# francescofugazzi/3dgsconverter

Hardware: NVIDIA H100
Metric: Msplats/s SOR k=16 (higher is better)
Workload: dtype f32

## Files before the change

3dgsconverter_b200/csrc/gsx_sor.cu:

```cuda
#include "gsx_common.cuh"
#include "gsx_sor.cuh"

#include "gsx_radix.cuh"
#include <math.h>

namespace gsx {

#define GSX_D2LIM_BITS 0x60ad78ebu
#define GSX_FULL 0xffffffffu

#ifndef GSX_MORTON_BITS
#define GSX_MORTON_BITS 15
#endif
constexpr int kMortonBits = GSX_MORTON_BITS;
constexpr float kMortonScale = (float)(1 << (GSX_MORTON_BITS / 3));
constexpr float kMortonMax = kMortonScale - 1.f;
#ifndef GSX_SMALL_BUCKET
#define GSX_SMALL_BUCKET 64
#endif
constexpr int kSmallBucket = GSX_SMALL_BUCKET;
#ifndef GSX_QUERY_BATCH
#define GSX_QUERY_BATCH 16
#endif
constexpr int kQueryBatch = GSX_QUERY_BATCH;
// ... 1004 lines not shown
                                : "memory");
                        }
                        bar_phase ^= 1u;
                        if (__all_sync(GSX_FULL, ok != 0)) {
                            staged_s = s13;
                            staged_c = c13;
                        }
                    }
                }
#endif
            }
            if (STATS) {
                int tot = pc;
#pragma unroll
                for (int o = 16; o > 0; o >>= 1) tot += __shfl_xor_sync(GSX_FULL, tot, o);
                st_visits += (unsigned long long)tot;
                st_queries += 1;
            }
            TopK<NREG> tk;
            tk.init(K);

            unsigned pkey = 0xffffffffu;
            if (pc > 0) {
                float dx = fmaxf(fmaxf(__fsub_rn(blx, q.x), __fsub_rn(q.x, bhx)), 0.f);
                float dy = fmaxf(fmaxf(__fsub_rn(bly, q.y), __fsub_rn(q.y, bhy)), 0.f);
                float dz = fmaxf(fmaxf(__fsub_rn(blz, q.z), __fsub_rn(q.z, bhz)), 0.f);
                pkey = __float_as_uint(__fadd_rn(__fadd_rn(__fmul_rn(dx, dx), __fmul_rn(dy, dy)), __fmul_rn(dz, dz)));
            }

            int skip_chunk = -1;
            {
                int s13 = __shfl_sync(GSX_FULL, ps, 13), c13 = __shfl_sync(GSX_FULL, pc, 13);
                if (c13 > kSmallBucket && i >= s13 && i < (pos_t)s13 + c13) {
                    skip_chunk = (int)(i >> 5);
                    const pos_t j = ((pos_t)skip_chunk << 5) + lane;
                    scan32<NREG, STATS>(spos, j, j >= s13 && j < (pos_t)s13 + c13, q.x, q.y, q.z, tk, lane,
                                        st_scanned);
                }
            }

#pragma unroll 1
            for (;;) {
                const unsigned mp = __reduce_min_sync(GSX_FULL, pkey);
                if (mp == 0xffffffffu || !(__uint_as_float(mp) < tk.tau)) break;
                const int p = __ffs(__ballot_sync(GSX_FULL, pkey == mp)) - 1;
                if (lane == p) pkey = 0xffffffffu;
                const int s = __shfl_sync(GSX_FULL, ps, p), c = __shfl_sync(GSX_FULL, pc, p);
                const pos_t e = (pos_t)s + c;
                if (c <= kSmallBucket) {
#if GSX_KNN_TMA
                    const bool from_smem = staged_c > 0 && s == staged_s;
#pragma unroll 1
                    for (pos_t base = s; base < e; base += 32)
                        scan32<NREG, STATS>(spos, base + lane, base + lane < e, q.x, q.y, q.z, tk, lane, st_scanned,
                                            from_smem ? wbuf + (base - s) : nullptr);
#else
#pragma unroll 1
                    for (pos_t base = s; base < e; base += 32)
                        scan32<NREG, STATS>(spos, base + lane, base + lane < e, q.x, q.y, q.z, tk, lane, st_scanned);
#endif
                    continue;
                }
                const int skip = p == 13 ? skip_chunk : -1;
                const int fc = s >> 5, lc = (int)((e - 1) >> 5);
                const int fs = fc >> 5, ls = lc >> 5;
                auto chunk_group = [&](const int cbase) {
                    const int cid = cbase + lane;
                    const bool cv = cid >= fc && cid <= lc && cid != skip;
                    unsigned ckey = 0xffffffffu;
                    if (cv) {
                        float lb = box_lb(caabb, cid, q.x, q.y, q.z);
                        if (lb < tk.tau) ckey = __float_as_uint(lb);
                    }
                    if (STATS) st_boxes += __popc(__ballot_sync(GSX_FULL, cv));
                    for (;;) {
                        unsigned mc = __reduce_min_sync(GSX_FULL, ckey);
                        if (mc == 0xffffffffu || !(__uint_as_float(mc) < tk.tau)) break;
                        int srcc = __ffs(__ballot_sync(GSX_FULL, ckey == mc)) - 1;
                        if (lane == srcc) ckey = 0xffffffffu;
                        const pos_t j = ((pos_t)(cbase + srcc) << 5) + lane;
                        scan32<NREG, STATS>(spos, j, j >= s && j < e, q.x, q.y, q.z, tk, lane, st_scanned);
                    }
                };
#if GSX_KNN_FLAT_SUPERS > 0
                if (ls - fs < GSX_KNN_FLAT_SUPERS) {
                    for (int cb = fc; cb <= lc; cb += 32) chunk_group(cb);
                    continue;
                }
#endif
                for (int sb = fs; sb <= ls; sb += 32) {
                    const int sid = sb + lane;
                    unsigned skey = 0xffffffffu;
                    if (sid <= ls) {
                        float lb = box_lb(saabb, sid, q.x, q.y, q.z);
                        if (lb < tk.tau) skey = __float_as_uint(lb);
                    }
                    if (STATS) st_boxes += __popc(__ballot_sync(GSX_FULL, sid <= ls));
                    for (;;) {
                        unsigned ms = __reduce_min_sync(GSX_FULL, skey);
                        if (ms == 0xffffffffu || !(__uint_as_float(ms) < tk.tau)) break;
                        int srcs = __ffs(__ballot_sync(GSX_FULL, skey == ms)) - 1;
                        if (lane == srcs) skey = 0xffffffffu;
                        chunk_group((sb + srcs) * 32);
                    }
                }
            }

            const float d0 = __fsqrt_rn(tk.v0), d1 = NREG == 2 ? __fsqrt_rn(tk.v1) : 0.f;
            if (ES > 0) {
                float* row = epi + (int)(i - qb_p) * ES;
                if (ES <= 32) {
                    if (lane < ES) row[lane] = lane == ES - 1 ? q.w : d0;
                } else {
                    row[lane] = d0;
                    if (lane == 0) row[ES - 1] = q.w;
                }
                continue;
            }
            int valid = __popc(__ballot_sync(GSX_FULL, lane < K && d0 < 0.9e10f));
            if (NREG == 2) valid += __popc(__ballot_sync(GSX_FULL, lane + 32 < K && d1 < 0.9e10f));
            float sum = 0.f;
            for (int r = 0; r < valid; ++r) {
                float x = (NREG == 2 && r >= 32) ? __shfl_sync(GSX_FULL, d1, r - 32) : __shfl_sync(GSX_FULL, d0, r);
                sum = __fadd_rn(sum, x);
            }
            if (lane == 0) final_means[__float_as_int(q.w)] = valid > 0 ? __fdiv_rn(sum, (float)valid) : 0.f;
        }
        if (ES > 0) {
            __syncwarp();
            if (lane < (int)(qe - qb)) {
                const float* row = epi + lane * ES;
                float sum = 0.f;
                int valid = 0;
                for (int r = 0; r < K; ++r) {
                    const float x = row[r];
                    if (x < 0.9e10f) {
                        sum = __fadd_rn(sum, x);
                        ++valid;
                    }
                }
                final_means[__float_as_int(row[ES - 1])] = valid > 0 ? __fdiv_rn(sum, (float)valid) : 0.f;
            }
            __syncwarp();
        }
    }
    if (STATS && lane == 0) {
        atomicAdd(stats + 0, st_visits);
        atomicAdd(stats + 1, st_scanned);
        atomicAdd(stats + 2, st_boxes);
        atomicAdd(stats + 3, st_queries);
    }
}

#ifndef GSX_KNN16
#define GSX_KNN16 0
#endif
#include "gsx_sor_knn16.cuh"

__global__ void k_fill_f32(float* p, int64_t n, float v) {
    int64_t i = (int64_t)blockIdx.x * blockDim.x + threadIdx.x;
    if (i < n) p[i] = v;
}

template <int NREG, bool STATS, int ES>
static int launch_knn(SorWs& w, int64_t q_begin, int64_t q_end, int q_stride, int q_phase, int K, int hash_mode,
                      const float* bmin, float cell,
                      float* final_means, unsigned long long* stats, uint64_t M, int64_t want, cudaStream_t st) {
    int per_sm = 0;
    const size_t smem = (size_t)8 * kQueryBatch * ES * sizeof(float);
    GSX_CUDA_CHECK(cudaOccupancyMaxActiveBlocksPerMultiprocessor(&per_sm, k_sor_knn<NREG, STATS, ES>, 256, smem));
    int64_t grid = (int64_t)sm_count() * (per_sm > 0 ? per_sm : 4);
    if (grid > want) grid = want;
    if (grid < 1) grid = 1;
    k_sor_knn<NREG, STATS, ES><<<(int)grid, 256, smem, st>>>(w.spos, w.tab_se, w.tab_box, w.cellbits, w.caabb, w.saabb, final_means, w.counters,
                                                      q_begin, q_end, q_stride, q_phase, K, hash_mode, bmin[0], bmin[1],
                                                      bmin[2], cell,
                                                      (uint32_t)w.n, M, stats);
    return GSX_OK;
}

template <bool STATS>
static int launch_knn16(SorWs& w, int64_t q_begin, int64_t q_end, int q_stride, int q_phase, int K, int hash_mode,
                        const float* bmin, float cell, float* final_means, unsigned long long* stats, uint64_t M,
                        int64_t want, cudaStream_t st) {
    int per_sm = 0;
    GSX_CUDA_CHECK(cudaOccupancyMaxActiveBlocksPerMultiprocessor(&per_sm, k_sor_knn16<STATS>, 256, 0));
    int64_t grid = (int64_t)sm_count() * (per_sm > 0 ? per_sm : 4);
    want = (want + 1) / 2;
    if (grid > want) grid = want;
    if (grid < 1) grid = 1;
    k_sor_knn16<STATS><<<(int)grid, 256, 0, st>>>(w.spos, w.tab_se, w.tab_box, w.cellbits, w.caabb, w.saabb, final_means,
                                                  w.counters, q_begin, q_end, q_stride, q_phase, K, hash_mode, bmin[0],
                                                  bmin[1], bmin[2], cell, (uint32_t)w.n, M, stats);
    return GSX_OK;
}

#define GSX_STR2(x) #x
#define GSX_STR(x) GSX_STR2(x)
#if GSX_KNN_FLAT_SUPERS > 0
#define GSX_FLAT_INFO ";flat_supers=" GSX_STR(GSX_KNN_FLAT_SUPERS)
#else
#define GSX_FLAT_INFO ""
#endif
const char* sor_build_info() {
    return "knn=r02c"
           ";epi_smem=" GSX_STR(GSX_KNN_EPI_SMEM) ";first_sort=" GSX_STR(GSX_KNN_FIRST_SORT)
           ";query_batch=" GSX_STR(GSX_QUERY_BATCH) ";minblocks=" GSX_STR(GSX_KNN_MINBLOCKS)
           ";merge_threshold=" GSX_STR(GSX_MERGE_THRESHOLD) ";small_bucket=" GSX_STR(GSX_SMALL_BUCKET)
           GSX_FLAT_INFO ";knn16=" GSX_STR(GSX_KNN16) ";tma=" GSX_STR(GSX_KNN_TMA) ";i32=" GSX_STR(GSX_KNN_I32);
}

int sor_mean_dists(SorWs& w, int64_t q_begin, int64_t q_end, int q_stride, int q_phase, int k, int hash_mode,
                   const float* bmin, float cell,
                   float* final_means, unsigned long long* stats, cudaStream_t st) {
    GSX_NVTX("gsx::sor_mean_dists(k_sor_knn)");
    int64_t n = w.n;
    GSX_REQUIRE(k >= 1, GSX_ERR_ARG, "sor: k must be >= 1 (got %d)", k);
    GSX_REQUIRE(hash_mode == 0 || hash_mode == 1, GSX_ERR_ARG, "sor: bad hash_mode %d", hash_mode);
    GSX_REQUIRE(q_begin >= 0 && q_end <= n && q_begin <= q_end, GSX_ERR_ARG, "sor: bad query range");
    GSX_REQUIRE(q_stride >= 1 && q_phase >= 0 && q_phase < q_stride, GSX_ERR_ARG, "sor: bad query stride/phase");
    int K = k < 50 ? k : 50;
    if (q_end == q_begin) return GSX_OK;
    if (!(cell > 1e-8f)) {
        GSX_REQUIRE(q_begin == 0 && q_end == n, GSX_ERR_UNSUPPORTED, "sor: degenerate cell with a query range");
        k_fill_f32<<<(int)((n + 255) / 256), 256, 0, st>>>(final_means, n, 0.f);
        GSX_KERNEL_CHECK();
        return GSX_OK;
    }
    GSX_CUDA_CHECK(cudaMemsetAsync(w.counters, 0, sizeof(unsigned int), st));
    uint64_t M = 0xFFFFFFFFFFFFFFFFull / (uint64_t)n + 1ull;
    int64_t nq = (q_end - q_begin + q_stride - 1) / q_stride + kQueryBatch;
    int64_t want = (nq + (int64_t)kQueryBatch * 8 - 1) / ((int64_t)kQueryBatch * 8);
    int rc;
    if (GSX_KNN16 && K <= 16)
        rc = stats ? launch_knn16<true>(w, q_begin, q_end, q_stride, q_phase, K, hash_mode, bmin, cell, final_means, stats, M, want, st)
                   : launch_knn16<false>(w, q_begin, q_end, q_stride, q_phase, K, hash_mode, bmin, cell, final_means, stats, M, want, st);
    else {
#define GSX_KNN_ARGS w, q_begin, q_end, q_stride, q_phase, K, hash_mode, bmin, cell, final_means, stats, M, want, st
        constexpr int ES16 = GSX_KNN_EPI_SMEM ? 17 : 0, ES32 = GSX_KNN_EPI_SMEM ? 33 : 0;
        if (K <= 16) rc = stats ? launch_knn<1, true, ES16>(GSX_KNN_ARGS) : launch_knn<1, false, ES16>(GSX_KNN_ARGS);
        else if (K <= 32) rc = stats ? launch_knn<1, true, ES32>(GSX_KNN_ARGS) : launch_knn<1, false, ES32>(GSX_KNN_ARGS);
        else rc = stats ? launch_knn<2, true, 0>(GSX_KNN_ARGS) : launch_knn<2, false, 0>(GSX_KNN_ARGS);
#undef GSX_KNN_ARGS
    }
    if (rc) return rc;
    GSX_KERNEL_CHECK();
    return GSX_OK;
}

}
```

3dgsconverter_b200/csrc/gsx_sor_knn16.cuh:

```cuda

#ifndef GSX_MERGE16_THRESHOLD
#define GSX_MERGE16_THRESHOLD 4
#endif
#ifndef GSX_KNN16_MINBLOCKS
#define GSX_KNN16_MINBLOCKS 6
#endif

struct Lanes16 {
    int base;
    int hl;
    __device__ __forceinline__ unsigned ballot(bool p) const { return (__ballot_sync(GSX_FULL, p) >> base) & 0xffffu; }
    template <class T>
    __device__ __forceinline__ T bcast(T x, int src_hl) const { return __shfl_sync(GSX_FULL, x, src_hl, 16); }
    __device__ __forceinline__ unsigned hmin(unsigned x, bool& either) const {
        const unsigned lo = __reduce_min_sync(GSX_FULL, base ? 0xffffffffu : x);
        const unsigned hi = __reduce_min_sync(GSX_FULL, base ? x : 0xffffffffu);
        either = (lo & hi) != 0xffffffffu;
        return base ? hi : lo;
    }
};

struct TopK16 {
    float v;
    float tau;
    int K;
    __device__ __forceinline__ void init(int k) {
        K = k;
        v = tau = __uint_as_float(GSX_D2LIM_BITS);
    }
    __device__ __forceinline__ void refresh_tau(const Lanes16& L) { tau = L.bcast(v, K - 1); }
    __device__ __forceinline__ void insert(float x, const Lanes16& L) {
        float up = __shfl_up_sync(GSX_FULL, v, 1, 16);
        if (L.hl == 0) up = 0.f;
        if (v > x) v = fmaxf(up, x);
    }
    __device__ __forceinline__ void merge16(float nv, const Lanes16& L) {
        const int hl = L.hl;
#pragma unroll
        for (int k = 2; k <= 16; k <<= 1) {
#pragma unroll
            for (int j = k >> 1; j > 0; j >>= 1) {
                const float o = __shfl_xor_sync(GSX_FULL, nv, j);
                nv = (((hl & k) == 0) == ((hl & j) == 0)) ? fminf(nv, o) : fmaxf(nv, o);
            }
        }
        const float r = L.bcast(nv, 15 - hl);
        float m = fminf(v, r);
#pragma unroll
        for (int j = 8; j > 0; j >>= 1) {
            const float o = __shfl_xor_sync(GSX_FULL, m, j);
            m = ((hl & j) == 0) ? fminf(m, o) : fmaxf(m, o);
        }
        v = m;
    }
};

template <bool STATS>
__device__ __forceinline__ void scan16(const float4* __restrict__ spos, pos_t j, bool valid, float qx, float qy, float qz,
                                       TopK16& tk, const Lanes16& L, unsigned long long& n_scanned) {
    const float sentinel = __uint_as_float(GSX_D2LIM_BITS);
    float d2 = sentinel;
    if (valid) {
        const float4 c = __ldg(spos + j);
        const float ax = __fsub_rn(qx, c.x), ay = __fsub_rn(qy, c.y), az = __fsub_rn(qz, c.z);
        d2 = __fadd_rn(__fadd_rn(__fmul_rn(ax, ax), __fmul_rn(ay, ay)), __fmul_rn(az, az));
    }
    if (STATS) n_scanned += __popc(L.ballot(valid));
    const bool pass = valid && d2 > 1.0e-12f && d2 < tk.tau;
    const unsigned mall = __ballot_sync(GSX_FULL, pass);
    if (!mall) return;
    unsigned mlo = mall & 0xffffu, mhi = mall >> 16;
    const bool mg_lo = __popc(mlo) >= GSX_MERGE16_THRESHOLD, mg_hi = __popc(mhi) >= GSX_MERGE16_THRESHOLD;
    if (mg_lo || mg_hi) {
        const bool domerge = L.base ? mg_hi : mg_lo;
        tk.merge16((domerge && pass) ? d2 : sentinel, L);
        if (mg_lo) mlo = 0u;
        if (mg_hi) mhi = 0u;
    }
    while (mlo | mhi) {
        const unsigned m = L.base ? mhi : mlo;
        float x = L.bcast(d2, m ? __ffs(m) - 1 : 0);
        if (!m) x = sentinel;
        mlo &= mlo - 1;
        mhi &= mhi - 1;
        tk.insert(x, L);
    }
    tk.refresh_tau(L);
}

template <bool STATS>
__global__ void __launch_bounds__(256, GSX_KNN16_MINBLOCKS)
    k_sor_knn16(const float4* __restrict__ spos, const int2* __restrict__ tab_se, const float4* __restrict__ tab_box,
                const uint32_t* __restrict__ cellbits, const float4* __restrict__ caabb, const float4* __restrict__ saabb,
                float* __restrict__ final_means, unsigned int* __restrict__ work, int64_t q_begin, int64_t q_end,
                int q_stride, int q_phase, int K, int hash_mode, float bx, float by, float bz, float cell, uint32_t n,
                uint64_t M, unsigned long long* __restrict__ stats) {
    static_assert(!GSX_KNN16 || kQueryBatch == 16, "a half-warp batch is one 16-position run");
    const int lane = lane_id();
    Lanes16 L;
    L.base = lane & 16;
    L.hl = lane & 15;
    const int hl = L.hl;
    unsigned long long st_visits = 0, st_scanned = 0, st_boxes = 0, st_queries = 0;
    const int p1 = hl + 16;
    const bool has1 = p1 < 27;
    const int dx0 = hl / 9 - 1, dy0 = (hl / 3) % 3 - 1, dz0 = hl % 3 - 1;
    const int dx1 = p1 / 9 - 1, dy1 = (p1 / 3) % 3 - 1, dz1 = p1 % 3 - 1;

    for (;;) {
        unsigned int b0 = 0;
        if (lane == 0) b0 = atomicAdd(work, 2u * (unsigned)kQueryBatch);
        b0 = __shfl_sync(GSX_FULL, b0, 0);
        const int64_t qb_lo = q_begin + ((int64_t)(b0 / kQueryBatch) * q_stride + q_phase) * kQueryBatch;
        if (qb_lo >= q_end) break;
        const int64_t qb64 = q_begin + ((int64_t)(b0 / kQueryBatch + (L.base >> 4)) * q_stride + q_phase) * kQueryBatch;
        const bool have = qb64 < q_end;
        const pos_t qb = have ? (pos_t)qb64 : 0;
        const int nq = !have ? 0 : (qb64 + kQueryBatch <= q_end ? kQueryBatch : (int)(q_end - qb64));
        int ps0 = 0, pc0 = 0, ps1 = 0, pc1 = 0;
        float l0x = 0.f, l0y = 0.f, l0z = 0.f, h0x = 0.f, h0y = 0.f, h0z = 0.f;
        float l1x = 0.f, l1y = 0.f, l1z = 0.f, h1x = 0.f, h1y = 0.f, h1z = 0.f;
#pragma unroll 1
        for (int t = 0; t < kQueryBatch; ++t) {
            const bool aq = t < nq;
            if (!__any_sync(GSX_FULL, aq)) break;
            const pos_t i = qb + t;
            float4 q = make_float4(0.f, 0.f, 0.f, 0.f);
            bool newcell = false;
            if (aq) {
                q = __ldg(spos + i);
                newcell = t == 0 || ((__ldg(cellbits + (i >> 5)) >> (i & 31)) & 1u);
            }
            if (__any_sync(GSX_FULL, newcell)) {
                const int gx = (int)floorf(__fdiv_rn(__fsub_rn(q.x, bx), cell));
                const int gy = (int)floorf(__fdiv_rn(__fsub_rn(q.y, by), cell));
                const int gz = (int)floorf(__fdiv_rn(__fsub_rn(q.z, bz), cell));
                if (newcell) {
                    const uint32_t h = probe_hash(gx + dx0, gy + dy0, gz + dz0, n, M, hash_mode);
                    const int2 se = __ldg(tab_se + h);
                    ps0 = se.x, pc0 = se.y - se.x;
                    if (pc0 > 0) {
                        const float4 a = __ldg(tab_box + 2 * (size_t)h), b = __ldg(tab_box + 2 * (size_t)h + 1);
                        l0x = a.x, l0y = a.y, l0z = a.z, h0x = b.x, h0y = b.y, h0z = b.z;
                    }
                    ps1 = 0, pc1 = 0;
                    if (has1) {
                        const uint32_t g = probe_hash(gx + dx1, gy + dy1, gz + dz1, n, M, hash_mode);
                        const int2 se1 = __ldg(tab_se + g);
                        ps1 = se1.x, pc1 = se1.y - se1.x;
                        if (pc1 > 0) {
                            const float4 a = __ldg(tab_box + 2 * (size_t)g), b = __ldg(tab_box + 2 * (size_t)g + 1);
                            l1x = a.x, l1y = a.y, l1z = a.z, h1x = b.x, h1y = b.y, h1z = b.z;
                        }
                    }
                }
            }
            if (STATS) {
                int tot = aq ? pc0 + pc1 : 0;
#pragma unroll
                for (int o = 8; o > 0; o >>= 1) tot += __shfl_xor_sync(GSX_FULL, tot, o);
                if (hl == 0 && aq) {
                    st_visits += (unsigned long long)tot;
                    st_queries += 1;
                }
            }
            TopK16 tk;
            tk.init(K);
            unsigned pk0 = 0xffffffffu, pk1 = 0xffffffffu;
            if (aq && pc0 > 0) {
                const float dx = fmaxf(fmaxf(__fsub_rn(l0x, q.x), __fsub_rn(q.x, h0x)), 0.f);
                const float dy = fmaxf(fmaxf(__fsub_rn(l0y, q.y), __fsub_rn(q.y, h0y)), 0.f);
                const float dz = fmaxf(fmaxf(__fsub_rn(l0z, q.z), __fsub_rn(q.z, h0z)), 0.f);
                pk0 = __float_as_uint(__fadd_rn(__fadd_rn(__fmul_rn(dx, dx), __fmul_rn(dy, dy)), __fmul_rn(dz, dz)));
            }
            if (aq && pc1 > 0) {
                const float dx = fmaxf(fmaxf(__fsub_rn(l1x, q.x), __fsub_rn(q.x, h1x)), 0.f);
                const float dy = fmaxf(fmaxf(__fsub_rn(l1y, q.y), __fsub_rn(q.y, h1y)), 0.f);
                const float dz = fmaxf(fmaxf(__fsub_rn(l1z, q.z), __fsub_rn(q.z, h1z)), 0.f);
                pk1 = __float_as_uint(__fadd_rn(__fadd_rn(__fmul_rn(dx, dx), __fmul_rn(dy, dy)), __fmul_rn(dz, dz)));
            }

            int skip_chunk = -1;
            {
                const int s13 = L.bcast(ps0, 13), c13 = L.bcast(pc0, 13);
                const bool seed = aq && c13 > kSmallBucket && i >= s13 && i < (pos_t)s13 + c13;
                if (__any_sync(GSX_FULL, seed)) {
                    if (seed) skip_chunk = (int)(i >> 5);
                    const pos_t j0 = ((pos_t)(i >> 5) << 5) + hl;
                    scan16<STATS>(spos, j0, seed && j0 >= s13 && j0 < (pos_t)s13 + c13, q.x, q.y, q.z, tk, L, st_scanned);
                    scan16<STATS>(spos, j0 + 16, seed && j0 + 16 >= s13 && j0 + 16 < (pos_t)s13 + c13, q.x, q.y, q.z, tk, L,
                                  st_scanned);
                }
            }

#pragma unroll 1
            for (;;) {
                const unsigned taub = __float_as_uint(tk.tau);
                unsigned mine = pk0 < pk1 ? pk0 : pk1;
                if (!(mine < taub)) mine = 0xffffffffu;
                bool either;
                const unsigned mp = L.hmin(mine, either);
                if (!either) break;
                const bool go = mp != 0xffffffffu;
                const unsigned holders = L.ballot(go && mine == mp);
                const int pl = holders ? __ffs(holders) - 1 : 0;
                const bool slot0 = pk0 == mp;
                const int s = L.bcast(slot0 ? ps0 : ps1, pl);
                int c = L.bcast(slot0 ? pc0 : pc1, pl);
                const bool centre = L.bcast((int)(slot0 && hl == 13), pl) != 0;
                if (go && hl == pl) {
                    if (slot0) pk0 = 0xffffffffu;
                    else pk1 = 0xffffffffu;
                }
                if (!go) c = 0;
                const pos_t e = (pos_t)s + c;
                const bool big = c > kSmallBucket;
                {
                    pos_t b = s;
                    const pos_t eb = big ? s : e;
#pragma unroll 1
                    while (__any_sync(GSX_FULL, b < eb)) {
                        scan16<STATS>(spos, b + hl, b + hl < eb, q.x, q.y, q.z, tk, L, st_scanned);
                        b += 16;
                    }
                }
                if (!__any_sync(GSX_FULL, big)) continue;
                const int skip = centre ? skip_chunk : -1;
                const int fc = s >> 5, lc = (int)((e - 1) >> 5);
                const int fs = big ? fc >> 5 : 1, ls = big ? lc >> 5 : 0;
                int sb = fs;
#pragma unroll 1
                while (__any_sync(GSX_FULL, sb <= ls)) {
                    const int sid = sb + hl;
                    const bool sv = sb <= ls && sid <= ls;
                    unsigned skey = 0xffffffffu;
                    if (sv) {
                        const float lb = box_lb(saabb, sid, q.x, q.y, q.z);
                        if (lb < tk.tau) skey = __float_as_uint(lb);
                    }
                    if (STATS) st_boxes += __popc(L.ballot(sv));
#pragma unroll 1
                    for (;;) {
                        if (!(skey < __float_as_uint(tk.tau))) skey = 0xffffffffu;
                        bool either_s;
                        const unsigned ms = L.hmin(skey, either_s);
                        if (!either_s) break;
                        const bool gos = ms != 0xffffffffu;
                        const unsigned sh = L.ballot(gos && skey == ms);
                        const int sl = sh ? __ffs(sh) - 1 : 0;
                        if (gos && hl == sl) skey = 0xffffffffu;
                        const int sup = sb + sl;
                        const int cid0 = sup * 32 + hl, cid1 = cid0 + 16;
                        const bool cv0 = gos && cid0 >= fc && cid0 <= lc && cid0 != skip;
                        const bool cv1 = gos && cid1 >= fc && cid1 <= lc && cid1 != skip;
                        unsigned ck0 = 0xffffffffu, ck1 = 0xffffffffu;
                        if (cv0) {
                            const float lb = box_lb(caabb, cid0, q.x, q.y, q.z);
                            if (lb < tk.tau) ck0 = __float_as_uint(lb);
                        }
                        if (cv1) {
                            const float lb = box_lb(caabb, cid1, q.x, q.y, q.z);
                            if (lb < tk.tau) ck1 = __float_as_uint(lb);
                        }
                        if (STATS) st_boxes += __popc(L.ballot(cv0)) + __popc(L.ballot(cv1));
#pragma unroll 1
                        for (;;) {
                            unsigned cmine = ck0 < ck1 ? ck0 : ck1;
                            if (!(cmine < __float_as_uint(tk.tau))) cmine = 0xffffffffu;
                            bool either_c;
                            const unsigned mc = L.hmin(cmine, either_c);
                            if (!either_c) break;
                            const bool goc = mc != 0xffffffffu;
                            const unsigned chh = L.ballot(goc && cmine == mc);
                            const int cl = chh ? __ffs(chh) - 1 : 0;
                            const bool cs0 = ck0 == mc;
                            const int chunk = L.bcast(cs0 ? cid0 : cid1, cl);
                            if (goc && hl == cl) {
                                if (cs0) ck0 = 0xffffffffu;
                                else ck1 = 0xffffffffu;
                            }
                            const pos_t j0 = ((pos_t)chunk << 5) + hl;
                            scan16<STATS>(spos, j0, goc && j0 >= s && j0 < e, q.x, q.y, q.z, tk, L, st_scanned);
                            scan16<STATS>(spos, j0 + 16, goc && j0 + 16 >= s && j0 + 16 < e, q.x, q.y, q.z, tk, L, st_scanned);
                        }
                    }
                    sb += 16;
                }
            }

            const float d = __fsqrt_rn(tk.v);
            const int valid = __popc(L.ballot(hl < K && d < 0.9e10f));
            float sum = 0.f;
#pragma unroll 1
            for (int r = 0; __any_sync(GSX_FULL, r < valid); ++r) {
                const float x = L.bcast(d, r & 15);
                if (r < valid) sum = __fadd_rn(sum, x);
            }
            if (aq && hl == 0) final_means[__float_as_int(q.w)] = valid > 0 ? __fdiv_rn(sum, (float)valid) : 0.f;
        }
    }
    if (STATS && hl == 0) {
        atomicAdd(stats + 0, st_visits);
        atomicAdd(stats + 1, st_scanned);
        atomicAdd(stats + 2, st_boxes);
        atomicAdd(stats + 3, st_queries);
    }
}
```

Baseline: 1098.

## Replace half-warp k16 kNN kernel with lane-per-query kernel using group box pruning

The half-warp cooperative top-16 kernel is replaced by a new kernel in which each lane owns one query and keeps its own register-resident sorted list of up to kLaneSlots distances. Warp-wide cell, super-chunk and chunk traversal is pruned with box-to-box lower bounds against the warp's query bounding box, and points are scanned through a shared tile. The aim is to remove per-query shuffle and ballot traffic and to share candidate loads across the 32 queries of a warp. In exchange it adds register pressure and divergence, since the warp visits the union of all its queries' candidates. The lane kernel is now the default for K at or below the slot count; before, the k16 path ran only when GSX_KNN16 was set, which defaulted to 0.

```diff
diff --git a/3dgsconverter_b200/csrc/gsx_sor.cu b/3dgsconverter_b200/csrc/gsx_sor.cu
--- a/3dgsconverter_b200/csrc/gsx_sor.cu
+++ b/3dgsconverter_b200/csrc/gsx_sor.cu
@@ -1180,10 +1180,7 @@
     }
 }
 
-#ifndef GSX_KNN16
-#define GSX_KNN16 0
-#endif
-#include "gsx_sor_knn16.cuh"
+#include "gsx_sor_knn_lane.cuh"
 
 __global__ void k_fill_f32(float* p, int64_t n, float v) {
     int64_t i = (int64_t)blockIdx.x * blockDim.x + threadIdx.x;
@@ -1208,18 +1205,18 @@
 }
 
 template <bool STATS>
-static int launch_knn16(SorWs& w, int64_t q_begin, int64_t q_end, int q_stride, int q_phase, int K, int hash_mode,
-                        const float* bmin, float cell, float* final_means, unsigned long long* stats, uint64_t M,
-                        int64_t want, cudaStream_t st) {
+static int launch_knn_lane(SorWs& w, int64_t q_begin, int64_t q_end, int q_stride, int q_phase, int K, int hash_mode,
+                           const float* bmin, float cell, float* final_means, unsigned long long* stats, uint64_t M,
+                           int64_t want, cudaStream_t st) {
     int per_sm = 0;
-    GSX_CUDA_CHECK(cudaOccupancyMaxActiveBlocksPerMultiprocessor(&per_sm, k_sor_knn16<STATS>, 256, 0));
+    GSX_CUDA_CHECK(cudaOccupancyMaxActiveBlocksPerMultiprocessor(&per_sm, k_sor_knn_lane<STATS>, 256, 0));
     int64_t grid = (int64_t)sm_count() * (per_sm > 0 ? per_sm : 4);
     want = (want + 1) / 2;
     if (grid > want) grid = want;
     if (grid < 1) grid = 1;
-    k_sor_knn16<STATS><<<(int)grid, 256, 0, st>>>(w.spos, w.tab_se, w.tab_box, w.cellbits, w.caabb, w.saabb, final_means,
-                                                  w.counters, q_begin, q_end, q_stride, q_phase, K, hash_mode, bmin[0],
-                                                  bmin[1], bmin[2], cell, (uint32_t)w.n, M, stats);
+    k_sor_knn_lane<STATS><<<(int)grid, 256, 0, st>>>(w.spos, w.tab_se, w.tab_box, w.cellbits, w.caabb, w.saabb,
+                                                     final_means, w.counters, q_begin, q_end, q_stride, q_phase, K,
+                                                     hash_mode, bmin[0], bmin[1], bmin[2], cell, (uint32_t)w.n, M, stats);
     return GSX_OK;
 }
 
@@ -1235,7 +1232,8 @@
            ";epi_smem=" GSX_STR(GSX_KNN_EPI_SMEM) ";first_sort=" GSX_STR(GSX_KNN_FIRST_SORT)
            ";query_batch=" GSX_STR(GSX_QUERY_BATCH) ";minblocks=" GSX_STR(GSX_KNN_MINBLOCKS)
            ";merge_threshold=" GSX_STR(GSX_MERGE_THRESHOLD) ";small_bucket=" GSX_STR(GSX_SMALL_BUCKET)
-           GSX_FLAT_INFO ";knn16=" GSX_STR(GSX_KNN16) ";tma=" GSX_STR(GSX_KNN_TMA) ";i32=" GSX_STR(GSX_KNN_I32);
+           GSX_FLAT_INFO ";k16=lane;lane_minblocks=" GSX_STR(GSX_KNN_LANE_MINBLOCKS) ";tma=" GSX_STR(GSX_KNN_TMA)
+           ";i32=" GSX_STR(GSX_KNN_I32);
 }
 
 int sor_mean_dists(SorWs& w, int64_t q_begin, int64_t q_end, int q_stride, int q_phase, int k, int hash_mode,
@@ -1260,17 +1258,12 @@
     int64_t nq = (q_end - q_begin + q_stride - 1) / q_stride + kQueryBatch;
     int64_t want = (nq + (int64_t)kQueryBatch * 8 - 1) / ((int64_t)kQueryBatch * 8);
     int rc;
-    if (GSX_KNN16 && K <= 16)
-        rc = stats ? launch_knn16<true>(w, q_begin, q_end, q_stride, q_phase, K, hash_mode, bmin, cell, final_means, stats, M, want, st)
-                   : launch_knn16<false>(w, q_begin, q_end, q_stride, q_phase, K, hash_mode, bmin, cell, final_means, stats, M, want, st);
-    else {
 #define GSX_KNN_ARGS w, q_begin, q_end, q_stride, q_phase, K, hash_mode, bmin, cell, final_means, stats, M, want, st
-        constexpr int ES16 = GSX_KNN_EPI_SMEM ? 17 : 0, ES32 = GSX_KNN_EPI_SMEM ? 33 : 0;
-        if (K <= 16) rc = stats ? launch_knn<1, true, ES16>(GSX_KNN_ARGS) : launch_knn<1, false, ES16>(GSX_KNN_ARGS);
-        else if (K <= 32) rc = stats ? launch_knn<1, true, ES32>(GSX_KNN_ARGS) : launch_knn<1, false, ES32>(GSX_KNN_ARGS);
-        else rc = stats ? launch_knn<2, true, 0>(GSX_KNN_ARGS) : launch_knn<2, false, 0>(GSX_KNN_ARGS);
+    constexpr int ES32 = GSX_KNN_EPI_SMEM ? 33 : 0;
+    if (K <= kLaneSlots) rc = stats ? launch_knn_lane<true>(GSX_KNN_ARGS) : launch_knn_lane<false>(GSX_KNN_ARGS);
+    else if (K <= 32) rc = stats ? launch_knn<1, true, ES32>(GSX_KNN_ARGS) : launch_knn<1, false, ES32>(GSX_KNN_ARGS);
+    else rc = stats ? launch_knn<2, true, 0>(GSX_KNN_ARGS) : launch_knn<2, false, 0>(GSX_KNN_ARGS);
 #undef GSX_KNN_ARGS
-    }
     if (rc) return rc;
     GSX_KERNEL_CHECK();
     return GSX_OK;
diff --git a/3dgsconverter_b200/csrc/gsx_sor_knn16.cuh b/3dgsconverter_b200/csrc/gsx_sor_knn16.cuh
--- a/3dgsconverter_b200/csrc/gsx_sor_knn16.cuh
+++ /dev/null
@@ -1,308 +0,0 @@
-
-#ifndef GSX_MERGE16_THRESHOLD
-#define GSX_MERGE16_THRESHOLD 4
-#endif
-#ifndef GSX_KNN16_MINBLOCKS
-#define GSX_KNN16_MINBLOCKS 6
-#endif
-
-struct Lanes16 {
-    int base;
-    int hl;
-    __device__ __forceinline__ unsigned ballot(bool p) const { return (__ballot_sync(GSX_FULL, p) >> base) & 0xffffu; }
-    template <class T>
-    __device__ __forceinline__ T bcast(T x, int src_hl) const { return __shfl_sync(GSX_FULL, x, src_hl, 16); }
-    __device__ __forceinline__ unsigned hmin(unsigned x, bool& either) const {
-        const unsigned lo = __reduce_min_sync(GSX_FULL, base ? 0xffffffffu : x);
-        const unsigned hi = __reduce_min_sync(GSX_FULL, base ? x : 0xffffffffu);
-        either = (lo & hi) != 0xffffffffu;
-        return base ? hi : lo;
-    }
-};
-
-struct TopK16 {
-    float v;
-    float tau;
-    int K;
-    __device__ __forceinline__ void init(int k) {
-        K = k;
-        v = tau = __uint_as_float(GSX_D2LIM_BITS);
-    }
-    __device__ __forceinline__ void refresh_tau(const Lanes16& L) { tau = L.bcast(v, K - 1); }
-    __device__ __forceinline__ void insert(float x, const Lanes16& L) {
-        float up = __shfl_up_sync(GSX_FULL, v, 1, 16);
-        if (L.hl == 0) up = 0.f;
-        if (v > x) v = fmaxf(up, x);
-    }
-    __device__ __forceinline__ void merge16(float nv, const Lanes16& L) {
-        const int hl = L.hl;
-#pragma unroll
-        for (int k = 2; k <= 16; k <<= 1) {
-#pragma unroll
-            for (int j = k >> 1; j > 0; j >>= 1) {
-                const float o = __shfl_xor_sync(GSX_FULL, nv, j);
-                nv = (((hl & k) == 0) == ((hl & j) == 0)) ? fminf(nv, o) : fmaxf(nv, o);
-            }
-        }
-        const float r = L.bcast(nv, 15 - hl);
-        float m = fminf(v, r);
-#pragma unroll
-        for (int j = 8; j > 0; j >>= 1) {
-            const float o = __shfl_xor_sync(GSX_FULL, m, j);
-            m = ((hl & j) == 0) ? fminf(m, o) : fmaxf(m, o);
-        }
-        v = m;
-    }
-};
-
-template <bool STATS>
-__device__ __forceinline__ void scan16(const float4* __restrict__ spos, pos_t j, bool valid, float qx, float qy, float qz,
-                                       TopK16& tk, const Lanes16& L, unsigned long long& n_scanned) {
-    const float sentinel = __uint_as_float(GSX_D2LIM_BITS);
-    float d2 = sentinel;
-    if (valid) {
-        const float4 c = __ldg(spos + j);
-        const float ax = __fsub_rn(qx, c.x), ay = __fsub_rn(qy, c.y), az = __fsub_rn(qz, c.z);
-        d2 = __fadd_rn(__fadd_rn(__fmul_rn(ax, ax), __fmul_rn(ay, ay)), __fmul_rn(az, az));
-    }
-    if (STATS) n_scanned += __popc(L.ballot(valid));
-    const bool pass = valid && d2 > 1.0e-12f && d2 < tk.tau;
-    const unsigned mall = __ballot_sync(GSX_FULL, pass);
-    if (!mall) return;
-    unsigned mlo = mall & 0xffffu, mhi = mall >> 16;
-    const bool mg_lo = __popc(mlo) >= GSX_MERGE16_THRESHOLD, mg_hi = __popc(mhi) >= GSX_MERGE16_THRESHOLD;
-    if (mg_lo || mg_hi) {
-        const bool domerge = L.base ? mg_hi : mg_lo;
-        tk.merge16((domerge && pass) ? d2 : sentinel, L);
-        if (mg_lo) mlo = 0u;
-        if (mg_hi) mhi = 0u;
-    }
-    while (mlo | mhi) {
-        const unsigned m = L.base ? mhi : mlo;
-        float x = L.bcast(d2, m ? __ffs(m) - 1 : 0);
-        if (!m) x = sentinel;
-        mlo &= mlo - 1;
-        mhi &= mhi - 1;
-        tk.insert(x, L);
-    }
-    tk.refresh_tau(L);
-}
-
-template <bool STATS>
-__global__ void __launch_bounds__(256, GSX_KNN16_MINBLOCKS)
-    k_sor_knn16(const float4* __restrict__ spos, const int2* __restrict__ tab_se, const float4* __restrict__ tab_box,
-                const uint32_t* __restrict__ cellbits, const float4* __restrict__ caabb, const float4* __restrict__ saabb,
-                float* __restrict__ final_means, unsigned int* __restrict__ work, int64_t q_begin, int64_t q_end,
-                int q_stride, int q_phase, int K, int hash_mode, float bx, float by, float bz, float cell, uint32_t n,
-                uint64_t M, unsigned long long* __restrict__ stats) {
-    static_assert(!GSX_KNN16 || kQueryBatch == 16, "a half-warp batch is one 16-position run");
-    const int lane = lane_id();
-    Lanes16 L;
-    L.base = lane & 16;
-    L.hl = lane & 15;
-    const int hl = L.hl;
-    unsigned long long st_visits = 0, st_scanned = 0, st_boxes = 0, st_queries = 0;
-    const int p1 = hl + 16;
-    const bool has1 = p1 < 27;
-    const int dx0 = hl / 9 - 1, dy0 = (hl / 3) % 3 - 1, dz0 = hl % 3 - 1;
-    const int dx1 = p1 / 9 - 1, dy1 = (p1 / 3) % 3 - 1, dz1 = p1 % 3 - 1;
-
-    for (;;) {
-        unsigned int b0 = 0;
-        if (lane == 0) b0 = atomicAdd(work, 2u * (unsigned)kQueryBatch);
-        b0 = __shfl_sync(GSX_FULL, b0, 0);
-        const int64_t qb_lo = q_begin + ((int64_t)(b0 / kQueryBatch) * q_stride + q_phase) * kQueryBatch;
-        if (qb_lo >= q_end) break;
-        const int64_t qb64 = q_begin + ((int64_t)(b0 / kQueryBatch + (L.base >> 4)) * q_stride + q_phase) * kQueryBatch;
-        const bool have = qb64 < q_end;
-        const pos_t qb = have ? (pos_t)qb64 : 0;
-        const int nq = !have ? 0 : (qb64 + kQueryBatch <= q_end ? kQueryBatch : (int)(q_end - qb64));
-        int ps0 = 0, pc0 = 0, ps1 = 0, pc1 = 0;
-        float l0x = 0.f, l0y = 0.f, l0z = 0.f, h0x = 0.f, h0y = 0.f, h0z = 0.f;
-        float l1x = 0.f, l1y = 0.f, l1z = 0.f, h1x = 0.f, h1y = 0.f, h1z = 0.f;
-#pragma unroll 1
-        for (int t = 0; t < kQueryBatch; ++t) {
-            const bool aq = t < nq;
-            if (!__any_sync(GSX_FULL, aq)) break;
-            const pos_t i = qb + t;
-            float4 q = make_float4(0.f, 0.f, 0.f, 0.f);
-            bool newcell = false;
-            if (aq) {
-                q = __ldg(spos + i);
-                newcell = t == 0 || ((__ldg(cellbits + (i >> 5)) >> (i & 31)) & 1u);
-            }
-            if (__any_sync(GSX_FULL, newcell)) {
-                const int gx = (int)floorf(__fdiv_rn(__fsub_rn(q.x, bx), cell));
-                const int gy = (int)floorf(__fdiv_rn(__fsub_rn(q.y, by), cell));
-                const int gz = (int)floorf(__fdiv_rn(__fsub_rn(q.z, bz), cell));
-                if (newcell) {
-                    const uint32_t h = probe_hash(gx + dx0, gy + dy0, gz + dz0, n, M, hash_mode);
-                    const int2 se = __ldg(tab_se + h);
-                    ps0 = se.x, pc0 = se.y - se.x;
-                    if (pc0 > 0) {
-                        const float4 a = __ldg(tab_box + 2 * (size_t)h), b = __ldg(tab_box + 2 * (size_t)h + 1);
-                        l0x = a.x, l0y = a.y, l0z = a.z, h0x = b.x, h0y = b.y, h0z = b.z;
-                    }
-                    ps1 = 0, pc1 = 0;
-                    if (has1) {
-                        const uint32_t g = probe_hash(gx + dx1, gy + dy1, gz + dz1, n, M, hash_mode);
-                        const int2 se1 = __ldg(tab_se + g);
-                        ps1 = se1.x, pc1 = se1.y - se1.x;
-                        if (pc1 > 0) {
-                            const float4 a = __ldg(tab_box + 2 * (size_t)g), b = __ldg(tab_box + 2 * (size_t)g + 1);
-                            l1x = a.x, l1y = a.y, l1z = a.z, h1x = b.x, h1y = b.y, h1z = b.z;
-                        }
-                    }
-                }
-            }
-            if (STATS) {
-                int tot = aq ? pc0 + pc1 : 0;
-#pragma unroll
-                for (int o = 8; o > 0; o >>= 1) tot += __shfl_xor_sync(GSX_FULL, tot, o);
-                if (hl == 0 && aq) {
-                    st_visits += (unsigned long long)tot;
-                    st_queries += 1;
-                }
-            }
-            TopK16 tk;
-            tk.init(K);
-            unsigned pk0 = 0xffffffffu, pk1 = 0xffffffffu;
-            if (aq && pc0 > 0) {
-                const float dx = fmaxf(fmaxf(__fsub_rn(l0x, q.x), __fsub_rn(q.x, h0x)), 0.f);
-                const float dy = fmaxf(fmaxf(__fsub_rn(l0y, q.y), __fsub_rn(q.y, h0y)), 0.f);
-                const float dz = fmaxf(fmaxf(__fsub_rn(l0z, q.z), __fsub_rn(q.z, h0z)), 0.f);
-                pk0 = __float_as_uint(__fadd_rn(__fadd_rn(__fmul_rn(dx, dx), __fmul_rn(dy, dy)), __fmul_rn(dz, dz)));
-            }
-            if (aq && pc1 > 0) {
-                const float dx = fmaxf(fmaxf(__fsub_rn(l1x, q.x), __fsub_rn(q.x, h1x)), 0.f);
-                const float dy = fmaxf(fmaxf(__fsub_rn(l1y, q.y), __fsub_rn(q.y, h1y)), 0.f);
-                const float dz = fmaxf(fmaxf(__fsub_rn(l1z, q.z), __fsub_rn(q.z, h1z)), 0.f);
-                pk1 = __float_as_uint(__fadd_rn(__fadd_rn(__fmul_rn(dx, dx), __fmul_rn(dy, dy)), __fmul_rn(dz, dz)));
-            }
-
-            int skip_chunk = -1;
-            {
-                const int s13 = L.bcast(ps0, 13), c13 = L.bcast(pc0, 13);
-                const bool seed = aq && c13 > kSmallBucket && i >= s13 && i < (pos_t)s13 + c13;
-                if (__any_sync(GSX_FULL, seed)) {
-                    if (seed) skip_chunk = (int)(i >> 5);
-                    const pos_t j0 = ((pos_t)(i >> 5) << 5) + hl;
-                    scan16<STATS>(spos, j0, seed && j0 >= s13 && j0 < (pos_t)s13 + c13, q.x, q.y, q.z, tk, L, st_scanned);
-                    scan16<STATS>(spos, j0 + 16, seed && j0 + 16 >= s13 && j0 + 16 < (pos_t)s13 + c13, q.x, q.y, q.z, tk, L,
-                                  st_scanned);
-                }
-            }
-
-#pragma unroll 1
-            for (;;) {
-                const unsigned taub = __float_as_uint(tk.tau);
-                unsigned mine = pk0 < pk1 ? pk0 : pk1;
-                if (!(mine < taub)) mine = 0xffffffffu;
-                bool either;
-                const unsigned mp = L.hmin(mine, either);
-                if (!either) break;
-                const bool go = mp != 0xffffffffu;
-                const unsigned holders = L.ballot(go && mine == mp);
-                const int pl = holders ? __ffs(holders) - 1 : 0;
-                const bool slot0 = pk0 == mp;
-                const int s = L.bcast(slot0 ? ps0 : ps1, pl);
-                int c = L.bcast(slot0 ? pc0 : pc1, pl);
-                const bool centre = L.bcast((int)(slot0 && hl == 13), pl) != 0;
-                if (go && hl == pl) {
-                    if (slot0) pk0 = 0xffffffffu;
-                    else pk1 = 0xffffffffu;
-                }
-                if (!go) c = 0;
-                const pos_t e = (pos_t)s + c;
-                const bool big = c > kSmallBucket;
-                {
-                    pos_t b = s;
-                    const pos_t eb = big ? s : e;
-#pragma unroll 1
-                    while (__any_sync(GSX_FULL, b < eb)) {
-                        scan16<STATS>(spos, b + hl, b + hl < eb, q.x, q.y, q.z, tk, L, st_scanned);
-                        b += 16;
-                    }
-                }
-                if (!__any_sync(GSX_FULL, big)) continue;
-                const int skip = centre ? skip_chunk : -1;
-                const int fc = s >> 5, lc = (int)((e - 1) >> 5);
-                const int fs = big ? fc >> 5 : 1, ls = big ? lc >> 5 : 0;
-                int sb = fs;
-#pragma unroll 1
-                while (__any_sync(GSX_FULL, sb <= ls)) {
-                    const int sid = sb + hl;
-                    const bool sv = sb <= ls && sid <= ls;
-                    unsigned skey = 0xffffffffu;
-                    if (sv) {
-                        const float lb = box_lb(saabb, sid, q.x, q.y, q.z);
-                        if (lb < tk.tau) skey = __float_as_uint(lb);
-                    }
-                    if (STATS) st_boxes += __popc(L.ballot(sv));
-#pragma unroll 1
-                    for (;;) {
-                        if (!(skey < __float_as_uint(tk.tau))) skey = 0xffffffffu;
-                        bool either_s;
-                        const unsigned ms = L.hmin(skey, either_s);
-                        if (!either_s) break;
-                        const bool gos = ms != 0xffffffffu;
-                        const unsigned sh = L.ballot(gos && skey == ms);
-                        const int sl = sh ? __ffs(sh) - 1 : 0;
-                        if (gos && hl == sl) skey = 0xffffffffu;
-                        const int sup = sb + sl;
-                        const int cid0 = sup * 32 + hl, cid1 = cid0 + 16;
-                        const bool cv0 = gos && cid0 >= fc && cid0 <= lc && cid0 != skip;
-                        const bool cv1 = gos && cid1 >= fc && cid1 <= lc && cid1 != skip;
-                        unsigned ck0 = 0xffffffffu, ck1 = 0xffffffffu;
-                        if (cv0) {
-                            const float lb = box_lb(caabb, cid0, q.x, q.y, q.z);
-                            if (lb < tk.tau) ck0 = __float_as_uint(lb);
-                        }
-                        if (cv1) {
-                            const float lb = box_lb(caabb, cid1, q.x, q.y, q.z);
-                            if (lb < tk.tau) ck1 = __float_as_uint(lb);
-                        }
-                        if (STATS) st_boxes += __popc(L.ballot(cv0)) + __popc(L.ballot(cv1));
-#pragma unroll 1
-                        for (;;) {
-                            unsigned cmine = ck0 < ck1 ? ck0 : ck1;
-                            if (!(cmine < __float_as_uint(tk.tau))) cmine = 0xffffffffu;
-                            bool either_c;
-                            const unsigned mc = L.hmin(cmine, either_c);
-                            if (!either_c) break;
-                            const bool goc = mc != 0xffffffffu;
-                            const unsigned chh = L.ballot(goc && cmine == mc);
-                            const int cl = chh ? __ffs(chh) - 1 : 0;
-                            const bool cs0 = ck0 == mc;
-                            const int chunk = L.bcast(cs0 ? cid0 : cid1, cl);
-                            if (goc && hl == cl) {
-                                if (cs0) ck0 = 0xffffffffu;
-                                else ck1 = 0xffffffffu;
-                            }
-                            const pos_t j0 = ((pos_t)chunk << 5) + hl;
-                            scan16<STATS>(spos, j0, goc && j0 >= s && j0 < e, q.x, q.y, q.z, tk, L, st_scanned);
-                            scan16<STATS>(spos, j0 + 16, goc && j0 + 16 >= s && j0 + 16 < e, q.x, q.y, q.z, tk, L, st_scanned);
-                        }
-                    }
-                    sb += 16;
-                }
-            }
-
-            const float d = __fsqrt_rn(tk.v);
-            const int valid = __popc(L.ballot(hl < K && d < 0.9e10f));
-            float sum = 0.f;
-#pragma unroll 1
-            for (int r = 0; __any_sync(GSX_FULL, r < valid); ++r) {
-                const float x = L.bcast(d, r & 15);
-                if (r < valid) sum = __fadd_rn(sum, x);
-            }
-            if (aq && hl == 0) final_means[__float_as_int(q.w)] = valid > 0 ? __fdiv_rn(sum, (float)valid) : 0.f;
-        }
-    }
-    if (STATS && hl == 0) {
-        atomicAdd(stats + 0, st_visits);
-        atomicAdd(stats + 1, st_scanned);
-        atomicAdd(stats + 2, st_boxes);
-        atomicAdd(stats + 3, st_queries);
-    }
-}
diff --git a/3dgsconverter_b200/csrc/gsx_sor_knn_lane.cuh b/3dgsconverter_b200/csrc/gsx_sor_knn_lane.cuh
--- /dev/null
+++ b/3dgsconverter_b200/csrc/gsx_sor_knn_lane.cuh
@@ -0,0 +1,256 @@
+
+#ifndef GSX_KNN_LANE_MINBLOCKS
+#define GSX_KNN_LANE_MINBLOCKS 4
+#endif
+constexpr int kLaneSlots = 16;
+
+__device__ __forceinline__ float boxbox_lb(float lx, float ly, float lz, float hx, float hy, float hz, float qlx,
+                                           float qly, float qlz, float qhx, float qhy, float qhz) {
+    const float dx = fmaxf(fmaxf(__fsub_rn(lx, qhx), __fsub_rn(qlx, hx)), 0.f);
+    const float dy = fmaxf(fmaxf(__fsub_rn(ly, qhy), __fsub_rn(qly, hy)), 0.f);
+    const float dz = fmaxf(fmaxf(__fsub_rn(lz, qhz), __fsub_rn(qlz, hz)), 0.f);
+    return __fadd_rn(__fadd_rn(__fmul_rn(dx, dx), __fmul_rn(dy, dy)), __fmul_rn(dz, dz));
+}
+
+template <bool STATS>
+__device__ __forceinline__ void lane_scan_tile(const float4* __restrict__ spos, float4* tile, pos_t a, int cnt, bool live,
+                                               const float4& q, float (&v)[kLaneSlots], int lane,
+                                               unsigned long long& n_scanned) {
+    if (lane < cnt) tile[lane] = __ldg(spos + a + lane);
+    __syncwarp();
+    if (STATS && live) n_scanned += (unsigned long long)cnt;
+#pragma unroll 2
+    for (int j = 0; j < cnt; ++j) {
+        const float4 c = tile[j];
+        const float ax = __fsub_rn(q.x, c.x), ay = __fsub_rn(q.y, c.y), az = __fsub_rn(q.z, c.z);
+        float x = __fadd_rn(__fadd_rn(__fmul_rn(ax, ax), __fmul_rn(ay, ay)), __fmul_rn(az, az));
+        if (live && x > 1.0e-12f && x < v[kLaneSlots - 1]) {
+#pragma unroll
+            for (int r = 0; r < kLaneSlots; ++r) {
+                const float lo = fminf(v[r], x);
+                x = fmaxf(v[r], x);
+                v[r] = lo;
+            }
+        }
+    }
+    __syncwarp();
+}
+
+__device__ __forceinline__ unsigned lane_run_taumax(bool act, const float (&v)[kLaneSlots]) {
+    return __reduce_max_sync(GSX_FULL, act ? __float_as_uint(v[kLaneSlots - 1]) : 0u);
+}
+
+template <bool STATS>
+__global__ void __launch_bounds__(256, STATS ? GSX_KNN_LANE_MINBLOCKS - 1 : GSX_KNN_LANE_MINBLOCKS)
+    k_sor_knn_lane(const float4* __restrict__ spos, const int2* __restrict__ tab_se, const float4* __restrict__ tab_box,
+                   const uint32_t* __restrict__ cellbits, const float4* __restrict__ caabb,
+                   const float4* __restrict__ saabb, float* __restrict__ final_means, unsigned int* __restrict__ work,
+                   int64_t q_begin, int64_t q_end, int q_stride, int q_phase, int K, int hash_mode, float bx, float by,
+                   float bz, float cell, uint32_t n, uint64_t M, unsigned long long* __restrict__ stats) {
+    static_assert(kQueryBatch == 16, "a warp takes two batches of 16 positions, one per half");
+    const int lane = lane_id();
+    __shared__ float4 s_tile[8][32];
+    float4* const tile = s_tile[threadIdx.x >> 5];
+    unsigned long long st_visits = 0, st_scanned = 0, st_boxes = 0, st_queries = 0;
+    const int pdx = lane / 9 - 1, pdy = (lane / 3) % 3 - 1, pdz = lane % 3 - 1;
+    const float sentinel = __uint_as_float(GSX_D2LIM_BITS);
+
+    for (;;) {
+        unsigned int b0 = 0;
+        if (lane == 0) b0 = atomicAdd(work, 2u * (unsigned)kQueryBatch);
+        b0 = __shfl_sync(GSX_FULL, b0, 0);
+        const int64_t bt = b0 / kQueryBatch;
+        if (q_begin + (bt * q_stride + q_phase) * kQueryBatch >= q_end) break;
+        const int64_t qi = q_begin + ((bt + (lane >> 4)) * q_stride + q_phase) * kQueryBatch + (lane & 15);
+        const bool has = qi < q_end;
+        const pos_t i = has ? (pos_t)qi : 0;
+        float4 q = make_float4(0.f, 0.f, 0.f, 0.f);
+        bool newcell = false;
+        if (has) {
+            q = __ldg(spos + i);
+            newcell = lane == 0 || (lane == 16 && q_stride != 1) || ((__ldg(cellbits + (i >> 5)) >> (i & 31)) & 1u);
+        }
+        unsigned runs = __ballot_sync(GSX_FULL, newcell);
+#pragma unroll 1
+        while (runs) {
+            const int r0 = __ffs(runs) - 1;
+            runs &= runs - 1;
+            const int r1 = runs ? __ffs(runs) - 1 : 32;
+            const bool act = has && lane >= r0 && lane < r1;
+
+            const float cx = __shfl_sync(GSX_FULL, q.x, r0), cy = __shfl_sync(GSX_FULL, q.y, r0),
+                        cz = __shfl_sync(GSX_FULL, q.z, r0);
+            int ps = 0, pc = 0;
+            float blx = 0.f, bly = 0.f, blz = 0.f, bhx = 0.f, bhy = 0.f, bhz = 0.f;
+            if (lane < 27) {
+                const int gx = (int)floorf(__fdiv_rn(__fsub_rn(cx, bx), cell));
+                const int gy = (int)floorf(__fdiv_rn(__fsub_rn(cy, by), cell));
+                const int gz = (int)floorf(__fdiv_rn(__fsub_rn(cz, bz), cell));
+                const uint32_t h = probe_hash(gx + pdx, gy + pdy, gz + pdz, n, M, hash_mode);
+                const int2 se = __ldg(tab_se + h);
+                ps = se.x;
+                pc = se.y - se.x;
+                if (pc > 0) {
+                    const float4 b0 = __ldg(tab_box + 2 * (size_t)h), b1 = __ldg(tab_box + 2 * (size_t)h + 1);
+                    blx = b0.x, bly = b0.y, blz = b0.z, bhx = b1.x, bhy = b1.y, bhz = b1.z;
+                }
+            }
+            if (STATS) {
+                int tot = pc;
+#pragma unroll
+                for (int o = 16; o > 0; o >>= 1) tot += __shfl_xor_sync(GSX_FULL, tot, o);
+                if (act) {
+                    st_visits += (unsigned long long)tot;
+                    st_queries += 1;
+                }
+            }
+            const float qlx = ord_to_float(__reduce_min_sync(GSX_FULL, act ? float_to_ord(q.x) : 0xffffffffu));
+            const float qly = ord_to_float(__reduce_min_sync(GSX_FULL, act ? float_to_ord(q.y) : 0xffffffffu));
+            const float qlz = ord_to_float(__reduce_min_sync(GSX_FULL, act ? float_to_ord(q.z) : 0xffffffffu));
+            const float qhx = ord_to_float(__reduce_max_sync(GSX_FULL, act ? float_to_ord(q.x) : 0u));
+            const float qhy = ord_to_float(__reduce_max_sync(GSX_FULL, act ? float_to_ord(q.y) : 0u));
+            const float qhz = ord_to_float(__reduce_max_sync(GSX_FULL, act ? float_to_ord(q.z) : 0u));
+
+            float v[kLaneSlots];
+#pragma unroll
+            for (int r = 0; r < kLaneSlots; ++r) v[r] = r < kLaneSlots - K ? -1.f : sentinel;
+
+            int skip0 = -1, skip1 = -1;
+            {
+                const int s13 = __shfl_sync(GSX_FULL, ps, 13), c13 = __shfl_sync(GSX_FULL, pc, 13);
+                if (c13 > kSmallBucket) {
+                    const pos_t e13 = (pos_t)s13 + c13;
+                    const unsigned in = __ballot_sync(GSX_FULL, act && i >= s13 && i < e13);
+                    if (in) {
+                        skip0 = (int)(__shfl_sync(GSX_FULL, i, __ffs(in) - 1) >> 5);
+                        skip1 = (int)(__shfl_sync(GSX_FULL, i, 31 - __clz(in)) >> 5);
+#pragma unroll 1
+                        for (int sc = skip0; sc <= skip1; ++sc) {
+                            const pos_t a = max((pos_t)sc << 5, (pos_t)s13), e = min(((pos_t)sc << 5) + 32, e13);
+                            lane_scan_tile<STATS>(spos, tile, a, (int)(e - a), act, q, v, lane, st_scanned);
+                        }
+                    }
+                }
+            }
+
+            unsigned tmax = lane_run_taumax(act, v);
+            unsigned pkey = 0xffffffffu;
+            if (pc > 0) pkey = __float_as_uint(boxbox_lb(blx, bly, blz, bhx, bhy, bhz, qlx, qly, qlz, qhx, qhy, qhz));
+
+            auto chunk_group = [&](const int cbase, const pos_t s, const pos_t e, const int fc, const int lc,
+                                   const int skA, const int skB) {
+                const int cid = cbase + lane;
+                const bool cv = cid >= fc && cid <= lc && cid != skA && cid != skB;
+                unsigned ckey = 0xffffffffu;
+                if (cv) {
+                    const float4 a = __ldg(caabb + 2 * cid), b = __ldg(caabb + 2 * cid + 1);
+                    const unsigned k = __float_as_uint(boxbox_lb(a.x, a.y, a.z, a.w, b.x, b.y, qlx, qly, qlz, qhx, qhy, qhz));
+                    if (k < tmax) ckey = k;
+                }
+                if (STATS) {
+                    const unsigned nb = __ballot_sync(GSX_FULL, cv);
+                    if (act) st_boxes += __popc(nb);
+                }
+#pragma unroll 1
+                for (;;) {
+                    const unsigned mc = __reduce_min_sync(GSX_FULL, ckey);
+                    if (!(mc < tmax)) break;
+                    const int src = __ffs(__ballot_sync(GSX_FULL, ckey == mc)) - 1;
+                    if (lane == src) ckey = 0xffffffffu;
+                    const int ch = cbase + src;
+                    const bool live = act && box_lb(caabb, ch, q.x, q.y, q.z) < v[kLaneSlots - 1];
+                    if (!__any_sync(GSX_FULL, live)) continue;
+                    const pos_t a = max((pos_t)ch << 5, s), ee = min(((pos_t)ch << 5) + 32, e);
+                    lane_scan_tile<STATS>(spos, tile, a, (int)(ee - a), live, q, v, lane, st_scanned);
+                    tmax = lane_run_taumax(act, v);
+                }
+            };
+
+#pragma unroll 1
+            for (;;) {
+                const unsigned mp = __reduce_min_sync(GSX_FULL, pkey);
+                if (!(mp < tmax)) break;
+                const int p = __ffs(__ballot_sync(GSX_FULL, pkey == mp)) - 1;
+                if (lane == p) pkey = 0xffffffffu;
+                const int s = __shfl_sync(GSX_FULL, ps, p), c = __shfl_sync(GSX_FULL, pc, p);
+                const float lb = boxbox_lb(__shfl_sync(GSX_FULL, blx, p), __shfl_sync(GSX_FULL, bly, p),
+                                           __shfl_sync(GSX_FULL, blz, p), __shfl_sync(GSX_FULL, bhx, p),
+                                           __shfl_sync(GSX_FULL, bhy, p), __shfl_sync(GSX_FULL, bhz, p), q.x, q.y, q.z,
+                                           q.x, q.y, q.z);
+                const pos_t e = (pos_t)s + c;
+                if (c <= kSmallBucket) {
+#pragma unroll 1
+                    for (pos_t base = s; base < e; base += 32) {
+                        const bool live = act && lb < v[kLaneSlots - 1];
+                        if (!__any_sync(GSX_FULL, live)) break;
+                        lane_scan_tile<STATS>(spos, tile, base, min(32, (int)(e - base)), live, q, v, lane, st_scanned);
+                    }
+                    tmax = lane_run_taumax(act, v);
+                    continue;
+                }
+                if (!__any_sync(GSX_FULL, act && lb < v[kLaneSlots - 1])) continue;
+                const int skA = p == 13 ? skip0 : -1, skB = p == 13 ? skip1 : -1;
+                const int fc = s >> 5, lc = (int)((e - 1) >> 5);
+                const int fs = fc >> 5, ls = lc >> 5;
+                if (GSX_KNN_FLAT_SUPERS > 0 && ls - fs < GSX_KNN_FLAT_SUPERS) {
+#pragma unroll 1
+                    for (int cb = fc; cb <= lc; cb += 32) chunk_group(cb, s, e, fc, lc, skA, skB);
+                    continue;
+                }
+#pragma unroll 1
+                for (int sb = fs; sb <= ls; sb += 32) {
+                    const int sid = sb + lane;
+                    unsigned skey = 0xffffffffu;
+                    if (sid <= ls) {
+                        const float4 a = __ldg(saabb + 2 * sid), b = __ldg(saabb + 2 * sid + 1);
+                        const unsigned k = __float_as_uint(boxbox_lb(a.x, a.y, a.z, a.w, b.x, b.y, qlx, qly, qlz, qhx, qhy, qhz));
+                        if (k < tmax) skey = k;
+                    }
+                    if (STATS) {
+                        const unsigned nb = __ballot_sync(GSX_FULL, sid <= ls);
+                        if (act) st_boxes += __popc(nb);
+                    }
+#pragma unroll 1
+                    for (;;) {
+                        const unsigned ms = __reduce_min_sync(GSX_FULL, skey);
+                        if (!(ms < tmax)) break;
+                        const int srcs = __ffs(__ballot_sync(GSX_FULL, skey == ms)) - 1;
+                        if (lane == srcs) skey = 0xffffffffu;
+                        if (!__any_sync(GSX_FULL, act && box_lb(saabb, sb + srcs, q.x, q.y, q.z) < v[kLaneSlots - 1]))
+                            continue;
+                        chunk_group((sb + srcs) * 32, s, e, fc, lc, skA, skB);
+                    }
+                }
+            }
+
+            if (act) {
+                float sum = 0.f;
+                int valid = 0;
+#pragma unroll
+                for (int r = 0; r < kLaneSlots; ++r) {
+                    const float d = __fsqrt_rn(v[r]);
+                    if (r >= kLaneSlots - K && d < 0.9e10f) {
+                        sum = __fadd_rn(sum, d);
+                        ++valid;
+                    }
+                }
+                final_means[__float_as_int(q.w)] = valid > 0 ? __fdiv_rn(sum, (float)valid) : 0.f;
+            }
+        }
+    }
+    if (STATS) {
+#pragma unroll
+        for (int o = 16; o > 0; o >>= 1) {
+            st_visits += __shfl_xor_sync(GSX_FULL, st_visits, o);
+            st_scanned += __shfl_xor_sync(GSX_FULL, st_scanned, o);
+            st_boxes += __shfl_xor_sync(GSX_FULL, st_boxes, o);
+            st_queries += __shfl_xor_sync(GSX_FULL, st_queries, o);
+        }
+    }
+    if (STATS && lane == 0) {
+        atomicAdd(stats + 0, st_visits);
+        atomicAdd(stats + 1, st_scanned);
+        atomicAdd(stats + 2, st_boxes);
+        atomicAdd(stats + 3, st_queries);
+    }
+}
```

Result: faster. 1227, median of 6 (+11.7%).
